# tpoisonooo/how-to-optimize-gemm

Measured on NVIDIA H100. Metric: SGEMM GFLOP/s (square N=4096 point of the 256..4096 sweep), higher is better.
Workload: dtype f16x2(scaled split-f32)

## Files before the change

how-to-optimize-gemm_b200/csrc/capi.cu:

```cuda
#include "../../include/b200gemm.h"

#include <cuda.h>
#include <cuda_runtime.h>
#include <stdio.h>
#include <stdlib.h>
#include <string.h>

#include <atomic>
#include <mutex>
#include <vector>

#include "gemm_ffma.cuh"
#include "gemm_generic.cuh"
#include "gemm_mxf4.cuh"
#include "gemm_tc.cuh"

using namespace b200;

namespace {

std::atomic<unsigned long long> g_launches{0};
int g_split_tail = 1;

struct KernelTimer {
// ... 29 lines not shown
    cudaError_t e;
    if ((e = cudaStreamCreateWithFlags(&h2d, cudaStreamNonBlocking)) != cudaSuccess) return e;
    if ((e = cudaStreamCreateWithFlags(&comp, cudaStreamNonBlocking)) != cudaSuccess) return e;
    if ((e = cudaStreamCreateWithFlags(&d2h, cudaStreamNonBlocking)) != cudaSuccess) return e;
    for (int i = 0; i < 8; i++) {
      if ((e = cudaEventCreateWithFlags(&in[i], cudaEventDisableTiming)) != cudaSuccess) return e;
      if ((e = cudaEventCreateWithFlags(&done[i], cudaEventDisableTiming)) != cudaSuccess) return e;
    }
    ready = true;
    return cudaSuccess;
  }
};
struct DevCtx {
  int ok = 0;
  int sms = 0;
  int dev = -1;
  int* flags = nullptr;
  unsigned flag_slot = 0;
  std::mutex ws_mu;
  Scratch ws;
  cudaEvent_t ws_event = nullptr;
  cudaStream_t ws_stream = nullptr;
  bool ws_busy = false;
  unsigned cmax_slot = 0;
  float* cmax_buf = nullptr;
  size_t cmax_cap = 0;
  int cmax_dirty[2] = {0, 0};
  cudaStream_t aux = nullptr;
  cudaEvent_t aux_fork = nullptr, aux_join = nullptr;
  std::mutex host_mu;
  Scratch scr[4];
  HostPipe pipe;
  std::vector<const void*> attr_done;
};
constexpr int kMaxDevices = 64;
DevCtx g_ctx[kMaxDevices];
std::mutex g_mu;

typedef CUresult (*EncodeTiledFn)(CUtensorMap*, CUtensorMapDataType, cuuint32_t, void*,
                                  const cuuint64_t*, const cuuint64_t*, const cuuint32_t*,
                                  const cuuint32_t*, CUtensorMapInterleave, CUtensorMapSwizzle,
                                  CUtensorMapL2promotion, CUtensorMapFloatOOBfill);
EncodeTiledFn g_encode = nullptr;

thread_local DevCtx* t_ctx = nullptr;

int ensure_device() {
  int dev = -1;
  if (cudaGetDevice(&dev) != cudaSuccess || dev < 0 || dev >= kMaxDevices) { cudaGetLastError(); t_ctx = nullptr; return B200_ERR_NO_DEVICE; }
  DevCtx* c = &g_ctx[dev];
  t_ctx = c;
  if (c->ok == 1) return 0;
// ... 76 lines not shown
  if (g_maps.size() < kMapCache) g_maps.push_back({key, m});
  else { g_maps[g_map_next] = {key, m}; g_map_next = (g_map_next + 1) % kMapCache; }
  *out = m;
  return 0;
}

inline bool aligned16(const void* p) { return (reinterpret_cast<uintptr_t>(p) & 15) == 0; }

int check_args(int m, int n, int k, const void* A, int lda, const void* B, int ldb, const void* C, int ldc) {
  if (m < 0 || n < 0 || k < 0) return B200_ERR_BAD_ARG;
  if (m == 0 || n == 0) return 1;
  if (!C || ldc < n) return B200_ERR_BAD_ARG;
  if (k > 0 && (!A || !B || lda < k || ldb < n)) return B200_ERR_BAD_ARG;
  return 0;
}

int last_launch_status() {
  cudaError_t e = cudaPeekAtLastError();
  if (e != cudaSuccess) { cudaGetLastError(); return (int)e; }
  return 0;
}

int g_pdl = 1;
int g_prepass_fork = 1;
template <typename... KArgs, typename... Args>
cudaError_t launch_pdl(void (*kern)(KArgs...), dim3 grid, dim3 block, size_t smem, cudaStream_t st, int cluster, Args&&... args) {
  cudaLaunchConfig_t cfg = {};
  cfg.gridDim = grid; cfg.blockDim = block; cfg.dynamicSmemBytes = smem; cfg.stream = st;
  cudaLaunchAttribute at[2];
  int n = 0;
  if (cluster > 1) {
    at[n].id = cudaLaunchAttributeClusterDimension;
    at[n].val.clusterDim.x = cluster; at[n].val.clusterDim.y = 1; at[n].val.clusterDim.z = 1;
    n++;
  }
  if (g_pdl) {
    at[n].id = cudaLaunchAttributeProgrammaticStreamSerialization;
    at[n].val.programmaticStreamSerializationAllowed = 1;
    n++;
  }
  cfg.attrs = at; cfg.numAttrs = n;
  return cudaLaunchKernelEx(&cfg, kern, std::forward<Args>(args)...);
}

template <typename T>
int launch_zero(int m, int n, T* C, int ldc, cudaStream_t st) {
  dim3 grid((n + 255) / 256, m < 4096 ? m : 4096);
// ... 223 lines not shown
  ws_acquire(st);
  struct Release { cudaStream_t s; ~Release() { ws_release(s); } } rel{st};
  uint16_t* pA = reinterpret_cast<uint16_t*>(t_ctx->ws.p);
  const uint16_t* pB = prepB ? prepB
                             : reinterpret_cast<uint16_t*>(reinterpret_cast<uint8_t*>(t_ctx->ws.p) + a_off);
  const SplitJob ja{A, lda, m, k, pA, pka, m}, jb{B, ldb, k, n, const_cast<uint16_t*>(pB), pnb, kp};
  int rc = launch_split<NP>(ja, jb, prepB ? 1 : 2, st);
  if (rc) return rc;
  if constexpr (NP == 3)
    return launch_tc<KIND_F16, 128, 4, float, ProdX3, 64>(m, n, k, pA, pka, NP * m, m, pB, pnb, NP * kp, kp, C, ldc, st, "tc_bf16x3_128x128", g_split_chunk_k[0], nullptr, nullptr, acc);
  else
    return launch_tc<KIND_F16, 128, 6, float, ProdX2, 64>(m, n, k, pA, pka, NP * m, m, pB, pnb, NP * kp, kp, C, ldc, st, "tc_bf16x2_128x128", g_split_chunk_k[1], nullptr, nullptr, acc);
}

struct F16Operand {
  const uint16_t* planes;
  long long pitch;
  int plane_rows;
  const float* maxv;
};
inline long long f16_pitch(int cols) { return ((long long)cols + 7) & ~7LL; }
inline int f16_b_rows(int k) { return (k + 31) & ~31; }

int launch_f16_split_rows(const float* A, long long lda, int rows, int cols, float* rmax, uint16_t* planes,
                          long long pitch, int plane_rows, cudaStream_t st) {
  int blocks = (plane_rows + 7) / 8;
  const int cap = t_ctx->sms * 16;
  if (blocks > cap) blocks = cap;
  if (blocks < 1) blocks = 1;
  if (cols <= 1024) launch_pdl(split_f16_rows_kernel<4>, dim3(blocks), dim3(256), 0, st, 1, A, (long long)lda, rows, cols, rmax, planes, pitch, plane_rows);
  else if (cols <= 2048) launch_pdl(split_f16_rows_kernel<8>, dim3(blocks), dim3(256), 0, st, 1, A, (long long)lda, rows, cols, rmax, planes, pitch, plane_rows);
  else if (cols <= 4096) launch_pdl(split_f16_rows_kernel<16>, dim3(blocks), dim3(256), 0, st, 1, A, (long long)lda, rows, cols, rmax, planes, pitch, plane_rows);
  else launch_pdl(split_f16_rows_kernel<0>, dim3(blocks), dim3(256), 0, st, 1, A, (long long)lda, rows, cols, rmax, planes, pitch, plane_rows);
  g_launches++;
  return last_launch_status();
}

int launch_f16_split_cols(const float* B, long long ldb, int rows, int cols, float* cmax, uint16_t* planes,
                          long long pitch, int plane_rows, float* zero_buf, int zero_n, cudaStream_t st) {
  launch_pdl(col_absmax_kernel, dim3((cols + 1023) / 1024, (rows + 15) / 16), dim3(256), 0, st, 1, B, (long long)ldb, rows, cols,
             reinterpret_cast<unsigned int*>(cmax));
  const int gx = (int)((pitch + 2047) / 2048);
  int gy = (t_ctx->sms * 8 + gx - 1) / gx;
  if (gy > (plane_rows + 1) / 2) gy = (plane_rows + 1) / 2;
  if (gy < 1) gy = 1;
  if (zero_buf && zero_n > gx * 2048) {
    cudaMemsetAsync(zero_buf, 0, (size_t)zero_n * 4, st);
    zero_buf = nullptr;
  }
  launch_pdl(split_f16_cols_kernel, dim3(gx, gy), dim3(256), 0, st, 1, B, (long long)ldb, rows, cols, (const float*)cmax, planes, pitch, plane_rows, zero_buf, zero_n);
  g_launches += 2;
  return last_launch_status();
}

int gemm_f16x2_core(int m, int n, int k, const F16Operand& a, const F16Operand& b, float* C, int ldc, int acc,
                    cudaStream_t st) {
  constexpr int NP = 2;
  return launch_tc<KIND_FP16, 128, 6, float, ProdX2, 64>(m, n, k, a.planes, a.pitch, NP * a.plane_rows, a.plane_rows,
                                                         b.planes, b.pitch, NP * b.plane_rows, b.plane_rows, C, ldc, st,
                                                         "tc_f16x2_128x128", g_split_chunk_k[2], a.maxv, b.maxv, acc);
}

int cmax_reserve(int n, float** cur, float** other, int* other_dirty) {
  DevCtx* c = t_ctx;
  if (c->cmax_cap < (size_t)n) {
    size_t cap = c->cmax_cap ? 2 * c->cmax_cap : 16384;
    if (cap < (size_t)n) cap = (size_t)n;
    if (c->cmax_buf) { cudaDeviceSynchronize(); cudaFree(c->cmax_buf); }
    c->cmax_buf = nullptr; c->cmax_cap = 0;
    cudaError_t e = cudaMalloc(&c->cmax_buf, 2 * cap * sizeof(float));
    if (e == cudaSuccess) e = cudaMemset(c->cmax_buf, 0, 2 * cap * sizeof(float));
    if (e != cudaSuccess) { cudaGetLastError(); return (int)e; }
    c->cmax_cap = cap;
    c->cmax_dirty[0] = c->cmax_dirty[1] = 0;
  }
  const unsigned slot = c->cmax_slot++ & 1u;
  *cur = c->cmax_buf + slot * c->cmax_cap;
  *other = c->cmax_buf + (slot ^ 1u) * c->cmax_cap;
  *other_dirty = c->cmax_dirty[slot ^ 1u];
  c->cmax_dirty[slot ^ 1u] = 0;
  c->cmax_dirty[slot] = n;
  return 0;
}

int gemm_f32_split_f16(int m, int n, int k, const float* A, int lda, const float* B, int ldb, float* C, int ldc,
                       cudaStream_t st, int acc = 0, const F16Operand* prepA = nullptr, const F16Operand* prepB = nullptr) {
  constexpr int NP = 2;
  const long long pka = f16_pitch(k), pnb = f16_pitch(n);
  const int kp = f16_b_rows(k);
  const size_t a_bytes = prepA ? 0 : (size_t)NP * m * pka * 2, b_bytes = prepB ? 0 : (size_t)NP * kp * pnb * 2;
  const size_t a_off = (a_bytes + 1023) & ~(size_t)1023;
  const size_t r_off = (a_off + b_bytes + 1023) & ~(size_t)1023;
  const size_t total = r_off + (prepA ? 0 : (size_t)m * 4);
  F16Operand oa, ob;
  if (prepA && prepB) return gemm_f16x2_core(m, n, k, *prepA, *prepB, C, ldc, acc, st);
  std::lock_guard<std::mutex> wlk(t_ctx->ws_mu);
  if (int rc = split_ws_reserve(total)) return rc;
  ws_acquire(st);
  struct Release { cudaStream_t s; ~Release() { ws_release(s); } } rel{st};
  uint8_t* base = reinterpret_cast<uint8_t*>(t_ctx->ws.p);
  DevCtx* c = t_ctx;
  const bool fork = !prepA && !prepB && g_prepass_fork && (double)m * k + (double)k * n >= 4.0e6;
  cudaStream_t sb = st;
  if (fork) {
    if (!c->aux) {
      if (cudaStreamCreateWithFlags(&c->aux, cudaStreamNonBlocking) != cudaSuccess ||
          cudaEventCreateWithFlags(&c->aux_fork, cudaEventDisableTiming) != cudaSuccess ||
          cudaEventCreateWithFlags(&c->aux_join, cudaEventDisableTiming) != cudaSuccess) { cudaGetLastError(); return B200_ERR_NO_DEVICE; }
    }
    cudaEventRecord(c->aux_fork, st);
    cudaStreamWaitEvent(c->aux, c->aux_fork, 0);
    sb = c->aux;
  }
  if (prepB) ob = *prepB;
  else {
    uint16_t* pB = reinterpret_cast<uint16_t*>(base + a_off);
    float *cmax, *other;
    int other_dirty;
    if (int rc = cmax_reserve(n, &cmax, &other, &other_dirty)) return rc;
    if (int rc = launch_f16_split_cols(B, ldb, k, n, cmax, pB, pnb, kp, other, other_dirty, sb)) return rc;
    ob = F16Operand{pB, pnb, kp, cmax};
  }
  if (prepA) oa = *prepA;
  else {
    uint16_t* pA = reinterpret_cast<uint16_t*>(base);
    float* rmax = reinterpret_cast<float*>(base + r_off);
    if (int rc = launch_f16_split_rows(A, lda, m, k, rmax, pA, pka, m, st)) return rc;
    oa = F16Operand{pA, pka, m, rmax};
  }
  if (fork) {
    cudaEventRecord(c->aux_join, c->aux);
    cudaStreamWaitEvent(st, c->aux_join, 0);
  }
  return gemm_f16x2_core(m, n, k, oa, ob, C, ldc, acc, st);
}

int launch_ffma(int m, int n, int k, const float* A, int lda, const float* B, int ldb, float* C, int ldc,
                int accumulate, cudaStream_t st) {
  using Cfg = FfmaCfg;
  CUtensorMap tmA, tmB;
  int rc = get_map(&tmA, A, CU_TENSOR_MAP_DATA_TYPE_FLOAT32, 4, k, m, (unsigned long long)lda * 4, Cfg::BK, Cfg::BM, 1);
  if (rc) return rc;
  rc = get_map(&tmB, B, CU_TENSOR_MAP_DATA_TYPE_FLOAT32, 4, n, k, (unsigned long long)ldb * 4, Cfg::BN, Cfg::BK, 0);
  if (rc) return rc;
  FfmaParams p;
  p.C = C; p.ldc = ldc; p.M = m; p.N = n; p.K = k;
  p.vec_ok = aligned16(C) && (ldc % 4) == 0;
  p.accumulate = accumulate;
  p.axpby = t_epi.axpby; p.alpha = t_epi.alpha; p.beta = t_epi.beta;
  p.tiles_m = (m + Cfg::BM - 1) / Cfg::BM;
  p.tiles_n = (n + Cfg::BN - 1) / Cfg::BN;
  p.group_m = 8;
  const int tiles = p.tiles_m * p.tiles_n, slots = 2 * t_ctx->sms;
  const int rem = tiles % slots;
  const bool halves = g_ffma_halves && rem > 0 && 2 * rem <= slots;
  p.full_tiles = halves ? tiles - rem : tiles;
// ... 96 lines not shown

int b200_gemm_device_ok(void) { return ensure_device(); }

const char* b200_gemm_strerror(int code) {
  switch (code) {
    case B200_OK: return "ok";
    case B200_ERR_BAD_ARG: return "bad argument";
    case B200_ERR_NO_DEVICE: return "no usable sm_90 CUDA device (there is no CPU fallback)";
    case B200_ERR_UNSUPPORTED: return "mode not supported for these operands";
    case B200_ERR_TENSORMAP: return "cuTensorMapEncodeTiled failed";
    case B200_ERR_NCCL: return "NCCL failure (b200_nccl_last_error has the text)";
    default: return code > 0 ? cudaGetErrorString((cudaError_t)code) : "unknown";
  }
}

const char* b200_gemm_last_kernel(void) { return t_last_kernel; }
unsigned long long b200_gemm_launch_count(void) { return g_launches.load(); }
int b200_gemm_default_f32_mode(void) { return resolve_f32_mode(B200_F32_AUTO); }
void b200_gemm_set_default_f32_mode(int mode) {
  if (mode >= 0 && mode != B200_F32_AUTO && mode <= B200_F32_F16X2) g_default_f32_mode.store(mode);
}
void b200_gemm_debug_set_b_desc(int lbo_bytes, int sbo_bytes) { g_dbg_b_lbo = lbo_bytes; g_dbg_b_sbo = sbo_bytes; }
void b200_gemm_debug_set_bn(int bn) { g_force_bn = bn; }
void b200_gemm_debug_set_pdl(int v) { g_pdl = (v & 1) != 0; g_prepass_fork = (v & 2) == 0; }
void b200_gemm_debug_set_dynamic_sched(int) {}
void b200_gemm_debug_set_cta_group(int) {}
void b200_gemm_debug_set_split_tail(int on) { g_split_tail = on; }
void b200_gemm_debug_set_epilogue(int) {}
void b200_gemm_debug_set_group_rows(int rows) { g_group_rows = rows; }
void b200_gemm_debug_set_ffma_variant(int v) { g_ffma_halves = v & 1; g_ffma_fat = v < 0 ? -1 : (v >> 1) & 1; }
void b200_gemm_debug_set_split_chunk(int x3_k, int x2_k) {
  g_split_chunk_k[0] = x3_k < 0 ? kSplitChunkDefault[0] : x3_k;
  g_split_chunk_k[1] = x2_k < 0 ? kSplitChunkDefault[1] : x2_k;
  g_split_chunk_k[2] = x2_k < 0 ? kSplitChunkDefault[2] : x2_k;
}
void b200_gemm_debug_kernel_timing(int enable) { g_ktimer.on = enable != 0; g_ktimer.n = 0; }
int b200_gemm_debug_kernel_time_ms(double* sum_ms) {
  double sum = 0;
  int cnt = 0;
  for (int i = 0; i < g_ktimer.n; i++) {
    float ms = 0.f;
    if (cudaEventSynchronize(g_ktimer.ev[i][1]) == cudaSuccess &&
        cudaEventElapsedTime(&ms, g_ktimer.ev[i][0], g_ktimer.ev[i][1]) == cudaSuccess) { sum += ms; cnt++; }
  }
  cudaGetLastError();
  g_ktimer.n = 0;
  if (sum_ms) *sum_ms = sum;
  return cnt;
}

int b200_gemm_reserve_workspace(size_t bytes) {
  int rc = ensure_device();
  if (rc) return rc;
  std::lock_guard<std::mutex> wlk(t_ctx->ws_mu);
  return split_ws_reserve(bytes);
}
size_t b200_gemm_workspace_bytes(int m, int n, int k, int precision_mode) {
  const int mode = resolve_f32_mode(precision_mode);
  if (m <= 0 || n <= 0 || k <= 0) return 0;
  if (mode == B200_F32_TF32) return (size_t)n * (size_t)(((long long)k + 3) & ~3LL) * 4;
  const int np = mode == B200_F32_BF16X3 ? 3 : (mode == B200_F32_BF16X2 || mode == B200_F32_F16X2) ? 2 : 0;
  if (!np) return 0;
  const size_t a = ((size_t)np * m * plane_pitch(k) * 2 + 1023) & ~(size_t)1023;
  const size_t b = ((size_t)np * b_plane_rows(k) * plane_pitch(n) * 2 + 1023) & ~(size_t)1023;
  return a + b + (size_t)m * 4 + 1024;
}

int b200_gemm_f32(int m, int n, int k, const float* dA, int lda, const float* dB, int ldb, float* dC,
                  int ldc, int precision_mode, void* stream) {
  return gemm_f32_impl(m, n, k, dA, lda, dB, ldb, dC, ldc, precision_mode, 0, (cudaStream_t)stream);
}

int b200_gemm_f32_ex(int m, int n, int k, float alpha, const float* dA, int lda, const float* dB, int ldb, float beta,
                     float* dC, int ldc, int precision_mode, void* stream) {
  cudaStream_t st = (cudaStream_t)stream;
  if (alpha == 1.f && beta == 0.f) return gemm_f32_impl(m, n, k, dA, lda, dB, ldb, dC, ldc, precision_mode, 0, st);
  if (alpha == 1.f && beta == 1.f) return gemm_f32_impl(m, n, k, dA, lda, dB, ldb, dC, ldc, precision_mode, 1, st);
  int rc = check_args(m, n, k, dA, lda, dB, ldb, dC, ldc);
  if (rc == 1) return 0;
  if (rc) return rc;
  rc = ensure_device();
  if (rc) return rc;
  if (alpha == 0.f || k == 0) {
    if (beta == 0.f) return launch_zero<float>(m, n, dC, ldc, st);
    const dim3 sg((n + 255) / 256, m < 4096 ? m : 4096);
    scale_inplace_kernel<<<sg, 256, 0, st>>>(m, n, dC, ldc, beta);
    g_launches++;
    return last_launch_status();
// ... 54 lines not shown
  float* maxv;
  int dev;
};
struct b200_packed_a : b200_packed {};
struct b200_packed_b : b200_packed {};

static int pack_operand(int side, int rows, int cols, const float* d, int ld, int precision_mode, b200_packed* h,
                        cudaStream_t st) {
  if (rows <= 0 || cols <= 0 || !d || ld < cols) return B200_ERR_BAD_ARG;
  const int mode = resolve_f32_mode(precision_mode);
  if (mode != B200_F32_F16X2 && (side != 1 || (mode != B200_F32_BF16X3 && mode != B200_F32_BF16X2))) return B200_ERR_UNSUPPORTED;
  int rc = ensure_device();
  if (rc) return rc;
  h->side = side; h->rows = rows; h->cols = cols; h->mode = mode; h->planes = nullptr; h->maxv = nullptr;
  h->dev = t_ctx->dev;
  if (mode == B200_F32_F16X2) {
    h->np = 2;
    h->pitch = f16_pitch(cols);
    h->plane_rows = side == 0 ? rows : f16_b_rows(rows);
    const size_t nmax = side == 0 ? (size_t)rows : (size_t)cols;
    cudaError_t e = cudaMalloc(&h->planes, (size_t)2 * h->plane_rows * h->pitch * 2);
    if (e == cudaSuccess) e = cudaMalloc(&h->maxv, nmax * 4);
    if (e != cudaSuccess) { cudaGetLastError(); return (int)e; }
    if (side == 0) return launch_f16_split_rows(d, ld, rows, cols, h->maxv, h->planes, h->pitch, h->plane_rows, st);
    e = cudaMemsetAsync(h->maxv, 0, nmax * 4, st);
    if (e != cudaSuccess) { cudaGetLastError(); return (int)e; }
    return launch_f16_split_cols(d, ld, rows, cols, h->maxv, h->planes, h->pitch, h->plane_rows, nullptr, 0, st);
  }
  h->np = mode == B200_F32_BF16X3 ? 3 : 2;
  h->pitch = plane_pitch(cols);
  h->plane_rows = b_plane_rows(rows);
  cudaError_t e = cudaMalloc(&h->planes, (size_t)h->np * h->plane_rows * h->pitch * 2);
  if (e != cudaSuccess) { cudaGetLastError(); return (int)e; }
  const SplitJob jb{d, ld, rows, cols, h->planes, h->pitch, h->plane_rows};
  return h->np == 3 ? launch_split<3>(jb, jb, 1, st) : launch_split<2>(jb, jb, 1, st);
}
static void pack_release(b200_packed* h) {
  if (!h) return;
  if (h->planes) cudaFree(h->planes);
  if (h->maxv) cudaFree(h->maxv);
}

int b200_gemm_f32_pack_b(int k, int n, const float* dB, int ldb, int precision_mode, b200_packed_b** out,
                         void* stream) {
  if (!out) return B200_ERR_BAD_ARG;
  *out = nullptr;
  b200_packed_b* h = new b200_packed_b();
  int rc = pack_operand(1, k, n, dB, ldb, precision_mode, h, (cudaStream_t)stream);
  t_last_kernel = "split_planes";
  if (rc) { pack_release(h); delete h; return rc; }
// ... 248 lines not shown
```

how-to-optimize-gemm_b200/csrc/gemm_tc.cuh:

```cuda
#pragma once
#include <cuda_fp16.h>
#include <string.h>
#include <type_traits>

#include "ptx.cuh"
#include "wgmma.cuh"

namespace b200 {

template <int KIND> struct KindTraits;
template <> struct KindTraits<KIND_F16>  { static constexpr int ELEM = 2; static constexpr bool B_KMAJOR = false; };
template <> struct KindTraits<KIND_FP16> { static constexpr int ELEM = 2; static constexpr bool B_KMAJOR = false; };
template <> struct KindTraits<KIND_TF32> { static constexpr int ELEM = 4; static constexpr bool B_KMAJOR = true; };
template <> struct KindTraits<KIND_I8>   { static constexpr int ELEM = 1; static constexpr bool B_KMAJOR = true; };

struct ProdSingle {
  static constexpr int N = 1, NPA = 1, NPB = 1;
  __host__ __device__ static constexpr int ia(int) { return 0; }
  __host__ __device__ static constexpr int ib(int) { return 0; }
};
struct ProdX3 {
  static constexpr int N = 6, NPA = 3, NPB = 3;
  __host__ __device__ static constexpr int ia(int i) { return i == 1 ? 2 : (i == 2 || i == 4) ? 1 : 0; }
  __host__ __device__ static constexpr int ib(int i) { return i == 0 ? 2 : (i == 2 || i == 3) ? 1 : 0; }
};
struct ProdX2 {
  static constexpr int N = 3, NPA = 2, NPB = 2;
  __host__ __device__ static constexpr int ia(int i) { return i == 1 ? 1 : 0; }
  __host__ __device__ static constexpr int ib(int i) { return i == 0 ? 1 : 0; }
};

// ... 427 lines not shown
        uint32_t w[4];
#pragma unroll
        for (int e = 0; e < 4; e++) w[e] = bf16_plane2(x[u][2 * e], x[u][2 * e + 1]);
        *reinterpret_cast<uint4*>(dst + ((long long)pl * plane_rows + r) * dld + c) = make_uint4(w[0], w[1], w[2], w[3]);
      }
    }
  }
}


__device__ __forceinline__ void split_f16x8(const float (&x)[8], uint4& h1, uint4& h2) {
  uint32_t a[4], b[4];
#pragma unroll
  for (int e = 0; e < 4; e++) {
    const __half2 p = __floats2half2_rn(x[2 * e], x[2 * e + 1]);
    const float2 pf = __half22float2(p);
    const __half2 q = __floats2half2_rn(x[2 * e] - pf.x, x[2 * e + 1] - pf.y);
    a[e] = *reinterpret_cast<const uint32_t*>(&p);
    b[e] = *reinterpret_cast<const uint32_t*>(&q);
  }
  h1 = make_uint4(a[0], a[1], a[2], a[3]);
  h2 = make_uint4(b[0], b[1], b[2], b[3]);
}
__device__ __forceinline__ void load8(const float* __restrict__ s, int c, int cols, bool vec, float (&x)[8]) {
  if (vec && c + 8 <= cols) {
    const float4 v0 = __ldg(reinterpret_cast<const float4*>(s + c));
    const float4 v1 = __ldg(reinterpret_cast<const float4*>(s + c) + 1);
    x[0] = v0.x; x[1] = v0.y; x[2] = v0.z; x[3] = v0.w;
    x[4] = v1.x; x[5] = v1.y; x[6] = v1.z; x[7] = v1.w;
  } else {
#pragma unroll
    for (int e = 0; e < 8; e++) x[e] = c + e < cols ? __ldg(s + c + e) : 0.f;
  }
}

template <int VPL>
__global__ void __launch_bounds__(256) split_f16_rows_kernel(const float* __restrict__ src, long long ld, int rows,
                                                             int cols, float* __restrict__ rmax,
                                                             uint16_t* __restrict__ dst, long long dld, int plane_rows) {
  griddep_launch();
  griddep_wait();
  const int lane = threadIdx.x & 31;
  const int nwarps = (gridDim.x * blockDim.x) >> 5;
  const bool vec = (ld & 3) == 0 && (reinterpret_cast<uintptr_t>(src) & 15) == 0;
  for (int r = (blockIdx.x * blockDim.x + threadIdx.x) >> 5; r < plane_rows; r += nwarps) {
    uint16_t* d1 = dst + (long long)r * dld;
    uint16_t* d2 = dst + ((long long)plane_rows + r) * dld;
    if (r >= rows) {
      for (int c = lane * 8; c < dld; c += 256) {
        *reinterpret_cast<uint4*>(d1 + c) = make_uint4(0, 0, 0, 0);
        *reinterpret_cast<uint4*>(d2 + c) = make_uint4(0, 0, 0, 0);
      }
      continue;
    }
    const float* s = src + (long long)r * ld;
    float mx = 0.f;
    if constexpr (VPL > 0) {
      float x[VPL][8];
#pragma unroll
      for (int j = 0; j < VPL; j++) {
        const int c = (j * 32 + lane) * 8;
#pragma unroll
        for (int e = 0; e < 8; e++) x[j][e] = 0.f;
        if (c < cols) load8(s, c, cols, vec, x[j]);
#pragma unroll
        for (int e = 0; e < 8; e++) mx = fmaxf(mx, fabsf(x[j][e]));
      }
#pragma unroll
      for (int o = 16; o > 0; o >>= 1) mx = fmaxf(mx, __shfl_xor_sync(0xffffffffu, mx, o));
      if (lane == 0) rmax[r] = mx;
      const int ex = -pow2_exp(mx);
#pragma unroll
      for (int j = 0; j < VPL; j++) {
        const int c = (j * 32 + lane) * 8;
        if (c < dld) {
#pragma unroll
          for (int e = 0; e < 8; e++) x[j][e] = scale_pow2(x[j][e], ex);
          uint4 h1, h2;
          split_f16x8(x[j], h1, h2);
          *reinterpret_cast<uint4*>(d1 + c) = h1;
          *reinterpret_cast<uint4*>(d2 + c) = h2;
        }
      }
    } else {
      for (int c0 = lane * 8; c0 < cols; c0 += 1024) {
        float x[4][8];
#pragma unroll
        for (int u = 0; u < 4; u++) {
          const int c = c0 + u * 256;
#pragma unroll
          for (int e = 0; e < 8; e++) x[u][e] = 0.f;
          if (c < cols) load8(s, c, cols, vec, x[u]);
#pragma unroll
          for (int e = 0; e < 8; e++) mx = fmaxf(mx, fabsf(x[u][e]));
        }
      }
#pragma unroll
      for (int o = 16; o > 0; o >>= 1) mx = fmaxf(mx, __shfl_xor_sync(0xffffffffu, mx, o));
      if (lane == 0) rmax[r] = mx;
      const int ex = -pow2_exp(mx);
      for (int c0 = lane * 8; c0 < dld; c0 += 512) {
        float x[2][8];
#pragma unroll
        for (int u = 0; u < 2; u++) {
          const int c = c0 + u * 256;
#pragma unroll
          for (int e = 0; e < 8; e++) x[u][e] = 0.f;
          if (c < cols) load8(s, c, cols, vec, x[u]);
        }
#pragma unroll
        for (int u = 0; u < 2; u++) {
          const int c = c0 + u * 256;
          if (c < dld) {
#pragma unroll
            for (int e = 0; e < 8; e++) x[u][e] = scale_pow2(x[u][e], ex);
            uint4 h1, h2;
            split_f16x8(x[u], h1, h2);
            *reinterpret_cast<uint4*>(d1 + c) = h1;
            *reinterpret_cast<uint4*>(d2 + c) = h2;
          }
        }
      }
    }
  }
}

__global__ void __launch_bounds__(256) col_absmax_kernel(const float* __restrict__ src, long long ld, int rows,
                                                         int cols, unsigned int* __restrict__ out) {
  constexpr int ROWS = 16;
  griddep_launch();
  griddep_wait();
  const int c = blockIdx.x * 1024 + threadIdx.x * 4;
  if (c >= cols) return;
  const int r0 = blockIdx.y * ROWS, r1 = min(r0 + ROWS, rows);
  const bool vec = (ld & 3) == 0 && (reinterpret_cast<uintptr_t>(src) & 15) == 0 && c + 4 <= cols;
  float4 mx = make_float4(0.f, 0.f, 0.f, 0.f);
  if (vec) {
#pragma unroll 16
    for (int r = r0; r < r1; r++) {
      const float4 v = __ldg(reinterpret_cast<const float4*>(src + (long long)r * ld + c));
      mx.x = fmaxf(mx.x, fabsf(v.x)); mx.y = fmaxf(mx.y, fabsf(v.y));
      mx.z = fmaxf(mx.z, fabsf(v.z)); mx.w = fmaxf(mx.w, fabsf(v.w));
    }
  } else {
    for (int r = r0; r < r1; r++) {
      const float* s = src + (long long)r * ld + c;
      mx.x = fmaxf(mx.x, fabsf(s[0]));
      if (c + 1 < cols) mx.y = fmaxf(mx.y, fabsf(s[1]));
      if (c + 2 < cols) mx.z = fmaxf(mx.z, fabsf(s[2]));
      if (c + 3 < cols) mx.w = fmaxf(mx.w, fabsf(s[3]));
    }
  }
  const float m4[4] = {mx.x, mx.y, mx.z, mx.w};
#pragma unroll
  for (int e = 0; e < 4; e++)
    if (c + e < cols && __float_as_uint(m4[e]) > __ldcg(out + c + e)) atomicMax(out + c + e, __float_as_uint(m4[e]));
}

__global__ void __launch_bounds__(256) split_f16_cols_kernel(const float* __restrict__ src, long long ld, int rows,
                                                             int cols, const float* __restrict__ cmax,
                                                             uint16_t* __restrict__ dst, long long dld, int plane_rows,
                                                             float* __restrict__ zero_buf, int zero_n) {
  griddep_launch();
  griddep_wait();
  const int c = (int)(blockIdx.x * 256 + threadIdx.x) * 8;
  if (blockIdx.y == 0 && zero_buf != nullptr) {
#pragma unroll
    for (int e = 0; e < 8; e++)
      if (c + e < zero_n) zero_buf[c + e] = 0.f;
  }
  if (c >= dld) return;
  const bool vec = (ld & 3) == 0 && (reinterpret_cast<uintptr_t>(src) & 15) == 0;
  int ex[8];
#pragma unroll
  for (int e = 0; e < 8; e++) ex[e] = c + e < cols ? -pow2_exp(__ldg(cmax + c + e)) : 0;
  for (int r0 = blockIdx.y * 2; r0 < plane_rows; r0 += gridDim.y * 2) {
    float x[2][8];
#pragma unroll
    for (int u = 0; u < 2; u++) {
      const int r = r0 + u;
#pragma unroll
      for (int e = 0; e < 8; e++) x[u][e] = 0.f;
      if (r < rows) load8(src + (long long)r * ld, c, cols, vec, x[u]);
    }
#pragma unroll
    for (int u = 0; u < 2; u++) {
      const int r = r0 + u;
      if (r >= plane_rows) break;
#pragma unroll
      for (int e = 0; e < 8; e++) x[u][e] = scale_pow2(x[u][e], ex[e]);
      uint4 h1, h2;
      split_f16x8(x[u], h1, h2);
      *reinterpret_cast<uint4*>(dst + (long long)r * dld + c) = h1;
      *reinterpret_cast<uint4*>(dst + ((long long)plane_rows + r) * dld + c) = h2;
    }
  }
}

}
```

how-to-optimize-gemm_b200/csrc/rowpanel.cuh:

```cuda
#pragma once
#include <dlfcn.h>
#include <nccl.h>

namespace {

struct NcclApi {
  void* lib = nullptr;
  bool ok = false;
  ncclResult_t (*Broadcast)(const void*, void*, size_t, ncclDataType_t, int, ncclComm_t, cudaStream_t) = nullptr;
  const char* (*GetErrorString)(ncclResult_t) = nullptr;
  ncclResult_t (*CommCount)(const ncclComm_t, int*) = nullptr;
  ncclResult_t (*CommUserRank)(const ncclComm_t, int*) = nullptr;
  ncclResult_t (*GetUniqueId)(ncclUniqueId*) = nullptr;
  ncclResult_t (*CommInitRank)(ncclComm_t*, int, ncclUniqueId, int) = nullptr;
  ncclResult_t (*CommDestroy)(ncclComm_t) = nullptr;
} g_nccl;
thread_local char t_nccl_err[256] = "";

int nccl_load(const char* path) {
  std::lock_guard<std::mutex> lk(g_mu);
  if (g_nccl.ok) return 0;
  const char* names[3] = {path, "libnccl.so.2", "libnccl.so"};
  for (int i = 0; i < 3 && !g_nccl.lib; i++)
    if (names[i] && names[i][0]) g_nccl.lib = dlopen(names[i], RTLD_NOW | RTLD_GLOBAL);
// ... 198 lines not shown
  for (int j = 0; j <= rp->nslices && j < cap; j++) bounds[j] = rp->k0[j];
  return rp->nslices;
}

int b200_gemm_f32_rowpanel(b200_rowpanel* rp, int m_local, int n, int k, const float* dA, int lda, float* dB,
                           int ldb, float* dC, int ldc, int root, void* stream) {
  if (!rp || n != rp->n || k != rp->k || m_local > rp->m_max || root < 0 || root >= rp->world) return B200_ERR_BAD_ARG;
  int rc = check_args(m_local, n, k, dA, lda, dB, ldb, dC, ldc);
  if (rc < 0) return rc;
  if (!dB || ldb < n) return B200_ERR_BAD_ARG;
  rc = ensure_device();
  if (rc) return rc;
  if (t_ctx->dev != rp->dev) return B200_ERR_BAD_ARG;
  cudaStream_t st = (cudaStream_t)stream;
  rp_mark(rp, 0, st);
  RP_CK(cudaEventRecord(rp->ev_start, st));
  RP_CK(cudaStreamWaitEvent(rp->comm_stream, rp->ev_start, 0));
  if ((rc = rowpanel_broadcast(rp, dB, ldb, n, root, nullptr))) return rc;
  if (m_local == 0) {
    RP_CK(cudaStreamWaitEvent(st, rp->ev_b[rp->nslices - 1], 0));
    return 0;
  }
  if (rp->mode == B200_F32_F16X2) {
    if ((rc = launch_f16_split_rows(dA, lda, m_local, k, rp->a_max, rp->a_planes, rp->a_pitch, m_local, st))) return rc;
    RP_CK(cudaMemsetAsync(rp->b_max, 0, (size_t)rp->nslices * n * 4, st));
    rp_mark(rp, 1, st);
    for (int j = 0; j < rp->nslices; j++) {
      const int kk0 = rp->k0[j], kr = rp->k0[j + 1] - kk0;
      RP_CK(cudaStreamWaitEvent(st, rp->ev_b[j], 0));
      rp_mark(rp, 8 + 6 * j + 2, st);
      float* cmax = rp->b_max + (size_t)j * n;
      if ((rc = launch_f16_split_cols(dB + (size_t)kk0 * ldb, ldb, kr, n, cmax, rp->b_planes[j], rp->b_pitch,
                                      rp->b_rows[j], nullptr, 0, st))) return rc;
      rp_mark(rp, 8 + 6 * j + 3, st);
      const F16Operand oa{rp->a_planes + kk0, rp->a_pitch, m_local, rp->a_max};
      const F16Operand ob{rp->b_planes[j], rp->b_pitch, rp->b_rows[j], cmax};
      const bool corun = rp->world > 1 && j + 1 < rp->nslices;
      t_sm_reserve = corun ? rp->reserve_sms : 0;
      rc = gemm_f16x2_core(m_local, n, kr, oa, ob, dC, ldc, j > 0 ? 1 : 0, st);
      t_sm_reserve = 0;
      if (rc) return rc;
      rp_mark(rp, 8 + 6 * j + 4, st);
    }
    return 0;
  }
  for (int j = 0; j < rp->nslices; j++) {
    const int kk0 = rp->k0[j], kr = rp->k0[j + 1] - kk0;
    RP_CK(cudaStreamWaitEvent(st, rp->ev_b[j], 0));
    const bool corun = rp->world > 1 && j + 1 < rp->nslices;
    t_sm_reserve = corun ? rp->reserve_sms : 0;
    rc = gemm_f32_impl(m_local, n, kr, dA + kk0, lda, dB + (size_t)kk0 * ldb, ldb, dC, ldc, rp->mode, j > 0 ? 1 : 0, st);
    t_sm_reserve = 0;
    if (rc) return rc;
  }
  return 0;
}
// ... 55 lines not shown
```

Baseline: 136,700.

## Fuse f16x2 split prepasses into one cluster kernel with smem tiles

Replaces the separate row-split kernel, column-absmax kernel (with atomics and double-buffered cmax memset) and column-split kernel, plus the aux-stream fork, with a single prepass kernel. A and B CTAs share one launch: B columns are split across an 8-CTA cluster that reduces column maxima through distributed shared memory, and each CTA stages its tile in shared memory via cp.async so the source is read once instead of twice. The aim is to cut launches, global reads and atomics in the prepass. In exchange it adds cluster synchronisation, reloads a tile when a slice exceeds the shared-memory buffer, and assumes B plane rows divide evenly by the cluster size.

Measured after the change: 138,700, median of 6. 1.4% higher.

```diff
diff --git a/how-to-optimize-gemm_b200/csrc/capi.cu b/how-to-optimize-gemm_b200/csrc/capi.cu
--- a/how-to-optimize-gemm_b200/csrc/capi.cu
+++ b/how-to-optimize-gemm_b200/csrc/capi.cu
@@ -75,12 +75,6 @@
   cudaEvent_t ws_event = nullptr;
   cudaStream_t ws_stream = nullptr;
   bool ws_busy = false;
-  unsigned cmax_slot = 0;
-  float* cmax_buf = nullptr;
-  size_t cmax_cap = 0;
-  int cmax_dirty[2] = {0, 0};
-  cudaStream_t aux = nullptr;
-  cudaEvent_t aux_fork = nullptr, aux_join = nullptr;
   std::mutex host_mu;
   Scratch scr[4];
   HostPipe pipe;
@@ -203,7 +197,6 @@
 }
 
 int g_pdl = 1;
-int g_prepass_fork = 1;
 template <typename... KArgs, typename... Args>
 cudaError_t launch_pdl(void (*kern)(KArgs...), dim3 grid, dim3 block, size_t smem, cudaStream_t st, int cluster, Args&&... args) {
   cudaLaunchConfig_t cfg = {};
@@ -473,34 +466,30 @@
 inline long long f16_pitch(int cols) { return ((long long)cols + 7) & ~7LL; }
 inline int f16_b_rows(int k) { return (k + 31) & ~31; }
 
-int launch_f16_split_rows(const float* A, long long lda, int rows, int cols, float* rmax, uint16_t* planes,
-                          long long pitch, int plane_rows, cudaStream_t st) {
-  int blocks = (plane_rows + 7) / 8;
-  const int cap = t_ctx->sms * 16;
-  if (blocks > cap) blocks = cap;
-  if (blocks < 1) blocks = 1;
-  if (cols <= 1024) launch_pdl(split_f16_rows_kernel<4>, dim3(blocks), dim3(256), 0, st, 1, A, (long long)lda, rows, cols, rmax, planes, pitch, plane_rows);
-  else if (cols <= 2048) launch_pdl(split_f16_rows_kernel<8>, dim3(blocks), dim3(256), 0, st, 1, A, (long long)lda, rows, cols, rmax, planes, pitch, plane_rows);
-  else if (cols <= 4096) launch_pdl(split_f16_rows_kernel<16>, dim3(blocks), dim3(256), 0, st, 1, A, (long long)lda, rows, cols, rmax, planes, pitch, plane_rows);
-  else launch_pdl(split_f16_rows_kernel<0>, dim3(blocks), dim3(256), 0, st, 1, A, (long long)lda, rows, cols, rmax, planes, pitch, plane_rows);
+int launch_f16_prepass(const F16SplitSide* a, const F16SplitSide* b, cudaStream_t st) {
+  F16PrepassParams p = {};
+  int a_ctas = 0;
+  if (b) {
+    p.b = *b;
+    p.b_rows_cta = b->plane_rows / kPrepassCluster;
+    const long long share = p.b_rows_cta;
+    p.b_w = share * 32 <= kPrepassTile && share * 64 > kPrepassTile ? 32 : 64;
+    p.b_ctas = kPrepassCluster * (int)((b->dld + p.b_w - 1) / p.b_w);
+  }
+  if (a) {
+    p.a = *a;
+    const long long fit = kPrepassTile / a->dld;
+    p.a_rows_cta = 1;
+    while (2 * p.a_rows_cta <= fit && 2 * p.a_rows_cta <= kPrepassThreads) p.a_rows_cta *= 2;
+    const int groups = (a->plane_rows + p.a_rows_cta - 1) / p.a_rows_cta;
+    a_ctas = (groups + kPrepassCluster - 1) / kPrepassCluster * kPrepassCluster;
+  }
+  constexpr int smem = kPrepassTile * 4;
+  if (int rc = ensure_smem_attr(f16x2_prepass_kernel, smem)) return rc;
+  cudaError_t e = launch_pdl(f16x2_prepass_kernel, dim3(p.b_ctas + a_ctas), dim3(kPrepassThreads), smem, st,
+                             kPrepassCluster, p);
+  if (e != cudaSuccess) { cudaGetLastError(); return (int)e; }
   g_launches++;
-  return last_launch_status();
-}
-
-int launch_f16_split_cols(const float* B, long long ldb, int rows, int cols, float* cmax, uint16_t* planes,
-                          long long pitch, int plane_rows, float* zero_buf, int zero_n, cudaStream_t st) {
-  launch_pdl(col_absmax_kernel, dim3((cols + 1023) / 1024, (rows + 15) / 16), dim3(256), 0, st, 1, B, (long long)ldb, rows, cols,
-             reinterpret_cast<unsigned int*>(cmax));
-  const int gx = (int)((pitch + 2047) / 2048);
-  int gy = (t_ctx->sms * 8 + gx - 1) / gx;
-  if (gy > (plane_rows + 1) / 2) gy = (plane_rows + 1) / 2;
-  if (gy < 1) gy = 1;
-  if (zero_buf && zero_n > gx * 2048) {
-    cudaMemsetAsync(zero_buf, 0, (size_t)zero_n * 4, st);
-    zero_buf = nullptr;
-  }
-  launch_pdl(split_f16_cols_kernel, dim3(gx, gy), dim3(256), 0, st, 1, B, (long long)ldb, rows, cols, (const float*)cmax, planes, pitch, plane_rows, zero_buf, zero_n);
-  g_launches += 2;
   return last_launch_status();
 }
 
@@ -510,28 +499,6 @@
   return launch_tc<KIND_FP16, 128, 6, float, ProdX2, 64>(m, n, k, a.planes, a.pitch, NP * a.plane_rows, a.plane_rows,
                                                          b.planes, b.pitch, NP * b.plane_rows, b.plane_rows, C, ldc, st,
                                                          "tc_f16x2_128x128", g_split_chunk_k[2], a.maxv, b.maxv, acc);
-}
-
-int cmax_reserve(int n, float** cur, float** other, int* other_dirty) {
-  DevCtx* c = t_ctx;
-  if (c->cmax_cap < (size_t)n) {
-    size_t cap = c->cmax_cap ? 2 * c->cmax_cap : 16384;
-    if (cap < (size_t)n) cap = (size_t)n;
-    if (c->cmax_buf) { cudaDeviceSynchronize(); cudaFree(c->cmax_buf); }
-    c->cmax_buf = nullptr; c->cmax_cap = 0;
-    cudaError_t e = cudaMalloc(&c->cmax_buf, 2 * cap * sizeof(float));
-    if (e == cudaSuccess) e = cudaMemset(c->cmax_buf, 0, 2 * cap * sizeof(float));
-    if (e != cudaSuccess) { cudaGetLastError(); return (int)e; }
-    c->cmax_cap = cap;
-    c->cmax_dirty[0] = c->cmax_dirty[1] = 0;
-  }
-  const unsigned slot = c->cmax_slot++ & 1u;
-  *cur = c->cmax_buf + slot * c->cmax_cap;
-  *other = c->cmax_buf + (slot ^ 1u) * c->cmax_cap;
-  *other_dirty = c->cmax_dirty[slot ^ 1u];
-  c->cmax_dirty[slot ^ 1u] = 0;
-  c->cmax_dirty[slot] = n;
-  return 0;
 }
 
 int gemm_f32_split_f16(int m, int n, int k, const float* A, int lda, const float* B, int ldb, float* C, int ldc,
@@ -542,47 +509,19 @@
   const size_t a_bytes = prepA ? 0 : (size_t)NP * m * pka * 2, b_bytes = prepB ? 0 : (size_t)NP * kp * pnb * 2;
   const size_t a_off = (a_bytes + 1023) & ~(size_t)1023;
   const size_t r_off = (a_off + b_bytes + 1023) & ~(size_t)1023;
-  const size_t total = r_off + (prepA ? 0 : (size_t)m * 4);
-  F16Operand oa, ob;
+  const size_t c_off = r_off + (prepA ? 0 : (size_t)m * 4);
+  const size_t total = c_off + (prepB ? 0 : (size_t)n * 4);
   if (prepA && prepB) return gemm_f16x2_core(m, n, k, *prepA, *prepB, C, ldc, acc, st);
   std::lock_guard<std::mutex> wlk(t_ctx->ws_mu);
   if (int rc = split_ws_reserve(total)) return rc;
   ws_acquire(st);
   struct Release { cudaStream_t s; ~Release() { ws_release(s); } } rel{st};
   uint8_t* base = reinterpret_cast<uint8_t*>(t_ctx->ws.p);
-  DevCtx* c = t_ctx;
-  const bool fork = !prepA && !prepB && g_prepass_fork && (double)m * k + (double)k * n >= 4.0e6;
-  cudaStream_t sb = st;
-  if (fork) {
-    if (!c->aux) {
-      if (cudaStreamCreateWithFlags(&c->aux, cudaStreamNonBlocking) != cudaSuccess ||
-          cudaEventCreateWithFlags(&c->aux_fork, cudaEventDisableTiming) != cudaSuccess ||
-          cudaEventCreateWithFlags(&c->aux_join, cudaEventDisableTiming) != cudaSuccess) { cudaGetLastError(); return B200_ERR_NO_DEVICE; }
-    }
-    cudaEventRecord(c->aux_fork, st);
-    cudaStreamWaitEvent(c->aux, c->aux_fork, 0);
-    sb = c->aux;
-  }
-  if (prepB) ob = *prepB;
-  else {
-    uint16_t* pB = reinterpret_cast<uint16_t*>(base + a_off);
-    float *cmax, *other;
-    int other_dirty;
-    if (int rc = cmax_reserve(n, &cmax, &other, &other_dirty)) return rc;
-    if (int rc = launch_f16_split_cols(B, ldb, k, n, cmax, pB, pnb, kp, other, other_dirty, sb)) return rc;
-    ob = F16Operand{pB, pnb, kp, cmax};
-  }
-  if (prepA) oa = *prepA;
-  else {
-    uint16_t* pA = reinterpret_cast<uint16_t*>(base);
-    float* rmax = reinterpret_cast<float*>(base + r_off);
-    if (int rc = launch_f16_split_rows(A, lda, m, k, rmax, pA, pka, m, st)) return rc;
-    oa = F16Operand{pA, pka, m, rmax};
-  }
-  if (fork) {
-    cudaEventRecord(c->aux_join, c->aux);
-    cudaStreamWaitEvent(st, c->aux_join, 0);
-  }
+  const F16SplitSide sa{A, lda, m, k, reinterpret_cast<uint16_t*>(base), pka, m, reinterpret_cast<float*>(base + r_off)};
+  const F16SplitSide sb{B, ldb, k, n, reinterpret_cast<uint16_t*>(base + a_off), pnb, kp, reinterpret_cast<float*>(base + c_off)};
+  if (int rc = launch_f16_prepass(prepA ? nullptr : &sa, prepB ? nullptr : &sb, st)) return rc;
+  const F16Operand oa = prepA ? *prepA : F16Operand{sa.dst, sa.dld, sa.plane_rows, sa.maxv};
+  const F16Operand ob = prepB ? *prepB : F16Operand{sb.dst, sb.dld, sb.plane_rows, sb.maxv};
   return gemm_f16x2_core(m, n, k, oa, ob, C, ldc, acc, st);
 }
 
@@ -725,7 +664,7 @@
 }
 void b200_gemm_debug_set_b_desc(int lbo_bytes, int sbo_bytes) { g_dbg_b_lbo = lbo_bytes; g_dbg_b_sbo = sbo_bytes; }
 void b200_gemm_debug_set_bn(int bn) { g_force_bn = bn; }
-void b200_gemm_debug_set_pdl(int v) { g_pdl = (v & 1) != 0; g_prepass_fork = (v & 2) == 0; }
+void b200_gemm_debug_set_pdl(int v) { g_pdl = (v & 1) != 0; }
 void b200_gemm_debug_set_dynamic_sched(int) {}
 void b200_gemm_debug_set_cta_group(int) {}
 void b200_gemm_debug_set_split_tail(int on) { g_split_tail = on; }
@@ -766,7 +705,7 @@
   if (!np) return 0;
   const size_t a = ((size_t)np * m * plane_pitch(k) * 2 + 1023) & ~(size_t)1023;
   const size_t b = ((size_t)np * b_plane_rows(k) * plane_pitch(n) * 2 + 1023) & ~(size_t)1023;
-  return a + b + (size_t)m * 4 + 1024;
+  return a + b + (size_t)m * 4 + (mode == B200_F32_F16X2 ? (size_t)n * 4 : 0) + 1024;
 }
 
 int b200_gemm_f32(int m, int n, int k, const float* dA, int lda, const float* dB, int ldb, float* dC,
@@ -867,10 +806,8 @@
     cudaError_t e = cudaMalloc(&h->planes, (size_t)2 * h->plane_rows * h->pitch * 2);
     if (e == cudaSuccess) e = cudaMalloc(&h->maxv, nmax * 4);
     if (e != cudaSuccess) { cudaGetLastError(); return (int)e; }
-    if (side == 0) return launch_f16_split_rows(d, ld, rows, cols, h->maxv, h->planes, h->pitch, h->plane_rows, st);
-    e = cudaMemsetAsync(h->maxv, 0, nmax * 4, st);
-    if (e != cudaSuccess) { cudaGetLastError(); return (int)e; }
-    return launch_f16_split_cols(d, ld, rows, cols, h->maxv, h->planes, h->pitch, h->plane_rows, nullptr, 0, st);
+    const F16SplitSide s{d, ld, rows, cols, h->planes, h->pitch, h->plane_rows, h->maxv};
+    return side == 0 ? launch_f16_prepass(&s, nullptr, st) : launch_f16_prepass(nullptr, &s, st);
   }
   h->np = mode == B200_F32_BF16X3 ? 3 : 2;
   h->pitch = plane_pitch(cols);
diff --git a/how-to-optimize-gemm_b200/csrc/gemm_tc.cuh b/how-to-optimize-gemm_b200/csrc/gemm_tc.cuh
--- a/how-to-optimize-gemm_b200/csrc/gemm_tc.cuh
+++ b/how-to-optimize-gemm_b200/csrc/gemm_tc.cuh
@@ -1,4 +1,5 @@
 #pragma once
+#include <cooperative_groups.h>
 #include <cuda_fp16.h>
 #include <string.h>
 #include <type_traits>
@@ -7,6 +8,8 @@
 #include "wgmma.cuh"
 
 namespace b200 {
+
+namespace cg = cooperative_groups;
 
 template <int KIND> struct KindTraits;
 template <> struct KindTraits<KIND_F16>  { static constexpr int ELEM = 2; static constexpr bool B_KMAJOR = false; };
@@ -480,179 +483,162 @@
   h1 = make_uint4(a[0], a[1], a[2], a[3]);
   h2 = make_uint4(b[0], b[1], b[2], b[3]);
 }
-__device__ __forceinline__ void load8(const float* __restrict__ s, int c, int cols, bool vec, float (&x)[8]) {
-  if (vec && c + 8 <= cols) {
-    const float4 v0 = __ldg(reinterpret_cast<const float4*>(s + c));
-    const float4 v1 = __ldg(reinterpret_cast<const float4*>(s + c) + 1);
-    x[0] = v0.x; x[1] = v0.y; x[2] = v0.z; x[3] = v0.w;
-    x[4] = v1.x; x[5] = v1.y; x[6] = v1.z; x[7] = v1.w;
+
+struct F16SplitSide {
+  const float* src; long long ld; int rows, cols;
+  uint16_t* dst; long long dld; int plane_rows;
+  float* maxv;
+};
+struct F16PrepassParams {
+  F16SplitSide a, b;
+  int b_ctas, b_w, b_rows_cta;
+  int a_rows_cta;
+};
+constexpr int kPrepassThreads = 256;
+constexpr int kPrepassCluster = 8;
+constexpr int kPrepassTile = 16384;
+
+__device__ __forceinline__ void cp_async16(uint32_t dst, const void* src, int bytes) {
+  asm volatile("cp.async.cg.shared.global [%0], [%1], 16, %2;" ::"r"(dst), "l"(src), "r"(bytes) : "memory");
+}
+__device__ __forceinline__ void cp_async4(uint32_t dst, const void* src, int bytes) {
+  asm volatile("cp.async.ca.shared.global [%0], [%1], 4, %2;" ::"r"(dst), "l"(src), "r"(bytes) : "memory");
+}
+
+__device__ __forceinline__ void prepass_load(const F16SplitSide& s, bool vec, int r0, int nr, int c0, int nc,
+                                             float* tile) {
+  const uint32_t t = smem_u32(tile);
+  if (vec) {
+    const int q = nc >> 2, n = nr * q;
+    for (int i = threadIdx.x; i < n; i += kPrepassThreads) {
+      const int r = i / q, c = c0 + 4 * (i - r * q), gr = r0 + r;
+      const int bytes = gr < s.rows ? 4 * min(max(s.cols - c, 0), 4) : 0;
+      cp_async16(t + 16 * i, bytes ? s.src + (long long)gr * s.ld + c : s.src, bytes);
+    }
   } else {
-#pragma unroll
-    for (int e = 0; e < 8; e++) x[e] = c + e < cols ? __ldg(s + c + e) : 0.f;
-  }
-}
-
-template <int VPL>
-__global__ void __launch_bounds__(256) split_f16_rows_kernel(const float* __restrict__ src, long long ld, int rows,
-                                                             int cols, float* __restrict__ rmax,
-                                                             uint16_t* __restrict__ dst, long long dld, int plane_rows) {
+    const int n = nr * nc;
+    for (int i = threadIdx.x; i < n; i += kPrepassThreads) {
+      const int r = i / nc, c = c0 + (i - r * nc), gr = r0 + r;
+      const bool in = gr < s.rows && c < s.cols;
+      cp_async4(t + 4 * i, in ? s.src + (long long)gr * s.ld + c : s.src, in ? 4 : 0);
+    }
+  }
+  asm volatile("cp.async.wait_all;" ::: "memory");
+  __syncthreads();
+}
+
+template <bool ROWS>
+__device__ __forceinline__ void prepass_store(const F16SplitSide& s, int r0, int nr, int c0, int nc, const float* tile,
+                                              const int* ex) {
+  const int q = nc >> 3, n = nr * q;
+  for (int i = threadIdx.x; i < n; i += kPrepassThreads) {
+    const int r = i / q, c = 8 * (i - r * q);
+    const float4 v0 = *reinterpret_cast<const float4*>(tile + r * nc + c);
+    const float4 v1 = *reinterpret_cast<const float4*>(tile + r * nc + c + 4);
+    float x[8] = {v0.x, v0.y, v0.z, v0.w, v1.x, v1.y, v1.z, v1.w};
+#pragma unroll
+    for (int e = 0; e < 8; e++) x[e] = scale_pow2(x[e], ROWS ? ex[r] : ex[c + e]);
+    uint4 h1, h2;
+    split_f16x8(x, h1, h2);
+    uint16_t* d = s.dst + (long long)(r0 + r) * s.dld + c0 + c;
+    *reinterpret_cast<uint4*>(d) = h1;
+    *reinterpret_cast<uint4*>(d + (long long)s.plane_rows * s.dld) = h2;
+  }
+}
+
+__global__ void __launch_bounds__(kPrepassThreads, 3) f16x2_prepass_kernel(const F16PrepassParams p) {
+  extern __shared__ float4 prepass_smem[];
+  float* tile = reinterpret_cast<float*>(prepass_smem);
+  __shared__ float red[kPrepassThreads];
+  __shared__ float part[64];
+  __shared__ int ex[kPrepassThreads];
   griddep_launch();
   griddep_wait();
-  const int lane = threadIdx.x & 31;
-  const int nwarps = (gridDim.x * blockDim.x) >> 5;
-  const bool vec = (ld & 3) == 0 && (reinterpret_cast<uintptr_t>(src) & 15) == 0;
-  for (int r = (blockIdx.x * blockDim.x + threadIdx.x) >> 5; r < plane_rows; r += nwarps) {
-    uint16_t* d1 = dst + (long long)r * dld;
-    uint16_t* d2 = dst + ((long long)plane_rows + r) * dld;
-    if (r >= rows) {
-      for (int c = lane * 8; c < dld; c += 256) {
-        *reinterpret_cast<uint4*>(d1 + c) = make_uint4(0, 0, 0, 0);
-        *reinterpret_cast<uint4*>(d2 + c) = make_uint4(0, 0, 0, 0);
-      }
-      continue;
-    }
-    const float* s = src + (long long)r * ld;
-    float mx = 0.f;
-    if constexpr (VPL > 0) {
-      float x[VPL][8];
-#pragma unroll
-      for (int j = 0; j < VPL; j++) {
-        const int c = (j * 32 + lane) * 8;
-#pragma unroll
-        for (int e = 0; e < 8; e++) x[j][e] = 0.f;
-        if (c < cols) load8(s, c, cols, vec, x[j]);
-#pragma unroll
-        for (int e = 0; e < 8; e++) mx = fmaxf(mx, fabsf(x[j][e]));
-      }
-#pragma unroll
-      for (int o = 16; o > 0; o >>= 1) mx = fmaxf(mx, __shfl_xor_sync(0xffffffffu, mx, o));
-      if (lane == 0) rmax[r] = mx;
-      const int ex = -pow2_exp(mx);
-#pragma unroll
-      for (int j = 0; j < VPL; j++) {
-        const int c = (j * 32 + lane) * 8;
-        if (c < dld) {
-#pragma unroll
-          for (int e = 0; e < 8; e++) x[j][e] = scale_pow2(x[j][e], ex);
-          uint4 h1, h2;
-          split_f16x8(x[j], h1, h2);
-          *reinterpret_cast<uint4*>(d1 + c) = h1;
-          *reinterpret_cast<uint4*>(d2 + c) = h2;
-        }
-      }
-    } else {
-      for (int c0 = lane * 8; c0 < cols; c0 += 1024) {
-        float x[4][8];
-#pragma unroll
-        for (int u = 0; u < 4; u++) {
-          const int c = c0 + u * 256;
-#pragma unroll
-          for (int e = 0; e < 8; e++) x[u][e] = 0.f;
-          if (c < cols) load8(s, c, cols, vec, x[u]);
-#pragma unroll
-          for (int e = 0; e < 8; e++) mx = fmaxf(mx, fabsf(x[u][e]));
-        }
-      }
-#pragma unroll
-      for (int o = 16; o > 0; o >>= 1) mx = fmaxf(mx, __shfl_xor_sync(0xffffffffu, mx, o));
-      if (lane == 0) rmax[r] = mx;
-      const int ex = -pow2_exp(mx);
-      for (int c0 = lane * 8; c0 < dld; c0 += 512) {
-        float x[2][8];
-#pragma unroll
-        for (int u = 0; u < 2; u++) {
-          const int c = c0 + u * 256;
-#pragma unroll
-          for (int e = 0; e < 8; e++) x[u][e] = 0.f;
-          if (c < cols) load8(s, c, cols, vec, x[u]);
-        }
-#pragma unroll
-        for (int u = 0; u < 2; u++) {
-          const int c = c0 + u * 256;
-          if (c < dld) {
-#pragma unroll
-            for (int e = 0; e < 8; e++) x[u][e] = scale_pow2(x[u][e], ex);
-            uint4 h1, h2;
-            split_f16x8(x[u], h1, h2);
-            *reinterpret_cast<uint4*>(d1 + c) = h1;
-            *reinterpret_cast<uint4*>(d2 + c) = h2;
-          }
-        }
-      }
-    }
-  }
-}
-
-__global__ void __launch_bounds__(256) col_absmax_kernel(const float* __restrict__ src, long long ld, int rows,
-                                                         int cols, unsigned int* __restrict__ out) {
-  constexpr int ROWS = 16;
-  griddep_launch();
-  griddep_wait();
-  const int c = blockIdx.x * 1024 + threadIdx.x * 4;
-  if (c >= cols) return;
-  const int r0 = blockIdx.y * ROWS, r1 = min(r0 + ROWS, rows);
-  const bool vec = (ld & 3) == 0 && (reinterpret_cast<uintptr_t>(src) & 15) == 0 && c + 4 <= cols;
-  float4 mx = make_float4(0.f, 0.f, 0.f, 0.f);
-  if (vec) {
-#pragma unroll 16
-    for (int r = r0; r < r1; r++) {
-      const float4 v = __ldg(reinterpret_cast<const float4*>(src + (long long)r * ld + c));
-      mx.x = fmaxf(mx.x, fabsf(v.x)); mx.y = fmaxf(mx.y, fabsf(v.y));
-      mx.z = fmaxf(mx.z, fabsf(v.z)); mx.w = fmaxf(mx.w, fabsf(v.w));
+  const int tid = threadIdx.x;
+  if ((int)blockIdx.x < p.b_ctas) {
+    const F16SplitSide& s = p.b;
+    cg::cluster_group cl = cg::this_cluster();
+    const int rank = (int)cl.block_rank();
+    const int W = p.b_w;
+    const int c0 = (blockIdx.x / kPrepassCluster) * W;
+    const int nc = (int)min((long long)W, s.dld - c0);
+    const int r0 = rank * p.b_rows_cta, r1 = r0 + p.b_rows_cta;
+    const int rt = kPrepassTile / W;
+    const int nt = (p.b_rows_cta + rt - 1) / rt;
+    const bool vec = (s.ld & 3) == 0 && (reinterpret_cast<uintptr_t>(s.src) & 15) == 0;
+    const int phases = kPrepassThreads / W, col = tid % W;
+    float m = 0.f;
+    for (int q = 0; q < nt; q++) {
+      const int tr0 = r0 + q * rt, tnr = min(rt, r1 - tr0);
+      if (q > 0) __syncthreads();
+      prepass_load(s, vec, tr0, tnr, c0, nc, tile);
+      if (col < nc)
+        for (int r = tid / W; r < tnr; r += phases) m = fmaxf(m, fabsf(tile[r * nc + col]));
+    }
+    red[tid] = m;
+    __syncthreads();
+    if (tid < W) {
+      float v = 0.f;
+      for (int i = 0; i < phases; i++) v = fmaxf(v, red[i * W + tid]);
+      part[tid] = v;
+    }
+    cl.sync();
+    if (tid < nc) {
+      float v = 0.f;
+      for (int q = 0; q < kPrepassCluster; q++) v = fmaxf(v, *cl.map_shared_rank(part + tid, q));
+      ex[tid] = -pow2_exp(v);
+      if (rank == 0 && c0 + tid < s.cols) s.maxv[c0 + tid] = v;
+    }
+    cl.sync();
+    for (int i = 0; i < nt; i++) {
+      const int q = (i + nt - 1) % nt;
+      const int tr0 = r0 + q * rt, tnr = min(rt, r1 - tr0);
+      if (i > 0) {
+        __syncthreads();
+        prepass_load(s, vec, tr0, tnr, c0, nc, tile);
+      }
+      prepass_store<false>(s, tr0, tnr, c0, nc, tile, ex);
     }
   } else {
-    for (int r = r0; r < r1; r++) {
-      const float* s = src + (long long)r * ld + c;
-      mx.x = fmaxf(mx.x, fabsf(s[0]));
-      if (c + 1 < cols) mx.y = fmaxf(mx.y, fabsf(s[1]));
-      if (c + 2 < cols) mx.z = fmaxf(mx.z, fabsf(s[2]));
-      if (c + 3 < cols) mx.w = fmaxf(mx.w, fabsf(s[3]));
-    }
-  }
-  const float m4[4] = {mx.x, mx.y, mx.z, mx.w};
-#pragma unroll
-  for (int e = 0; e < 4; e++)
-    if (c + e < cols && __float_as_uint(m4[e]) > __ldcg(out + c + e)) atomicMax(out + c + e, __float_as_uint(m4[e]));
-}
-
-__global__ void __launch_bounds__(256) split_f16_cols_kernel(const float* __restrict__ src, long long ld, int rows,
-                                                             int cols, const float* __restrict__ cmax,
-                                                             uint16_t* __restrict__ dst, long long dld, int plane_rows,
-                                                             float* __restrict__ zero_buf, int zero_n) {
-  griddep_launch();
-  griddep_wait();
-  const int c = (int)(blockIdx.x * 256 + threadIdx.x) * 8;
-  if (blockIdx.y == 0 && zero_buf != nullptr) {
-#pragma unroll
-    for (int e = 0; e < 8; e++)
-      if (c + e < zero_n) zero_buf[c + e] = 0.f;
-  }
-  if (c >= dld) return;
-  const bool vec = (ld & 3) == 0 && (reinterpret_cast<uintptr_t>(src) & 15) == 0;
-  int ex[8];
-#pragma unroll
-  for (int e = 0; e < 8; e++) ex[e] = c + e < cols ? -pow2_exp(__ldg(cmax + c + e)) : 0;
-  for (int r0 = blockIdx.y * 2; r0 < plane_rows; r0 += gridDim.y * 2) {
-    float x[2][8];
-#pragma unroll
-    for (int u = 0; u < 2; u++) {
-      const int r = r0 + u;
-#pragma unroll
-      for (int e = 0; e < 8; e++) x[u][e] = 0.f;
-      if (r < rows) load8(src + (long long)r * ld, c, cols, vec, x[u]);
-    }
-#pragma unroll
-    for (int u = 0; u < 2; u++) {
-      const int r = r0 + u;
-      if (r >= plane_rows) break;
-#pragma unroll
-      for (int e = 0; e < 8; e++) x[u][e] = scale_pow2(x[u][e], ex[e]);
-      uint4 h1, h2;
-      split_f16x8(x[u], h1, h2);
-      *reinterpret_cast<uint4*>(dst + (long long)r * dld + c) = h1;
-      *reinterpret_cast<uint4*>(dst + ((long long)plane_rows + r) * dld + c) = h2;
-    }
-  }
-}
-
-}
+    const F16SplitSide& s = p.a;
+    const int G = p.a_rows_cta;
+    const int g0 = ((int)blockIdx.x - p.b_ctas) * G;
+    if (g0 >= s.plane_rows) return;
+    const int nr = min(G, s.plane_rows - g0);
+    const int tw = (int)min(s.dld, (long long)kPrepassTile);
+    const int nt = (int)((s.dld + tw - 1) / tw);
+    const bool vec = (s.ld & 3) == 0 && (reinterpret_cast<uintptr_t>(s.src) & 15) == 0;
+    const int tpr = kPrepassThreads / G, j = tid / tpr;
+    float m = 0.f;
+    for (int q = 0; q < nt; q++) {
+      const int tc0 = q * tw, tnc = (int)min((long long)tw, s.dld - tc0);
+      if (q > 0) __syncthreads();
+      prepass_load(s, vec, g0, nr, tc0, tnc, tile);
+      if (j < nr)
+        for (int c = tid % tpr; c < tnc; c += tpr) m = fmaxf(m, fabsf(tile[j * tnc + c]));
+    }
+    const int w = min(tpr, 32);
+    for (int o = w / 2; o > 0; o >>= 1) m = fmaxf(m, __shfl_xor_sync(0xffffffffu, m, o));
+    if (tid % w == 0) red[tid / w] = m;
+    __syncthreads();
+    if (tid < nr) {
+      const int per = tpr / w;
+      float v = 0.f;
+      for (int i = 0; i < per; i++) v = fmaxf(v, red[tid * per + i]);
+      ex[tid] = -pow2_exp(v);
+      if (g0 + tid < s.rows) s.maxv[g0 + tid] = v;
+    }
+    __syncthreads();
+    for (int i = 0; i < nt; i++) {
+      const int q = (i + nt - 1) % nt;
+      const int tc0 = q * tw, tnc = (int)min((long long)tw, s.dld - tc0);
+      if (i > 0) {
+        __syncthreads();
+        prepass_load(s, vec, g0, nr, tc0, tnc, tile);
+      }
+      prepass_store<true>(s, g0, nr, tc0, tnc, tile, ex);
+    }
+  }
+}
+
+}
diff --git a/how-to-optimize-gemm_b200/csrc/rowpanel.cuh b/how-to-optimize-gemm_b200/csrc/rowpanel.cuh
--- a/how-to-optimize-gemm_b200/csrc/rowpanel.cuh
+++ b/how-to-optimize-gemm_b200/csrc/rowpanel.cuh
@@ -244,16 +244,16 @@
     return 0;
   }
   if (rp->mode == B200_F32_F16X2) {
-    if ((rc = launch_f16_split_rows(dA, lda, m_local, k, rp->a_max, rp->a_planes, rp->a_pitch, m_local, st))) return rc;
-    RP_CK(cudaMemsetAsync(rp->b_max, 0, (size_t)rp->nslices * n * 4, st));
+    const F16SplitSide sa{dA, lda, m_local, k, rp->a_planes, rp->a_pitch, m_local, rp->a_max};
+    if ((rc = launch_f16_prepass(&sa, nullptr, st))) return rc;
     rp_mark(rp, 1, st);
     for (int j = 0; j < rp->nslices; j++) {
       const int kk0 = rp->k0[j], kr = rp->k0[j + 1] - kk0;
       RP_CK(cudaStreamWaitEvent(st, rp->ev_b[j], 0));
       rp_mark(rp, 8 + 6 * j + 2, st);
       float* cmax = rp->b_max + (size_t)j * n;
-      if ((rc = launch_f16_split_cols(dB + (size_t)kk0 * ldb, ldb, kr, n, cmax, rp->b_planes[j], rp->b_pitch,
-                                      rp->b_rows[j], nullptr, 0, st))) return rc;
+      const F16SplitSide sb{dB + (size_t)kk0 * ldb, ldb, kr, n, rp->b_planes[j], rp->b_pitch, rp->b_rows[j], cmax};
+      if ((rc = launch_f16_prepass(nullptr, &sb, st))) return rc;
       rp_mark(rp, 8 + 6 * j + 3, st);
       const F16Operand oa{rp->a_planes + kk0, rp->a_pitch, m_local, rp->a_max};
       const F16Operand ob{rp->b_planes[j], rp->b_pitch, rp->b_rows[j], cmax};
```
